# mlnoga/nightlight

Measured on AMD Instinct MI355X. Metric: stacked Mpixels/sec (sigma-clip, 128x4096x4096 fp32), higher is better.
Workload: dtype f32

## Files before the change

nightlight_amd/csrc/fast_common.hpp:

```cpp
#pragma once
#include <type_traits>
#include <utility>

#include "stack_kernels.h"

namespace nl {

constexpr float kU = 5.9604644775390625e-8f;
constexpr int kZone = 8;
constexpr int kPadMax = 8;
constexpr unsigned kGenericGrid = 2048;
inline unsigned generic_grid(unsigned hint, unsigned pixels_per_wg, unsigned max_grid)
{
    if (hint == 0) return max_grid;
    const unsigned need = (hint - 1 + pixels_per_wg - 1) / pixels_per_wg;
    const unsigned g = need + need / 2 + 64;
    return g < max_grid ? g : max_grid;
}

__device__ __forceinline__ void snapshot_fb_list(const FastArgs &q)
{
    if (q.fb_snap && threadIdx.x == 0 && __atomic_load_n(q.fb_snap, __ATOMIC_RELAXED) == 0u) {
        const unsigned len = __atomic_load_n(q.fb_count, __ATOMIC_RELAXED);
        const unsigned prev = atomicCAS(q.fb_snap, 0u, len + 1u);
        if (prev == 0xffffffffu) __builtin_trap();
        __threadfence();
    }
    __syncthreads();
}

__device__ __forceinline__ void fused_prologue_dominant(const StackArgs &p)
{
    if (p.zero_next && blockIdx.x == 0) {
        for (int i = threadIdx.x; i < kScratchWords; i += blockDim.x) p.zero_next[i] = 0ull;
        if (threadIdx.x < 4) p.final[threadIdx.x] = 0ull;
    }
}
__device__ __forceinline__ void fused_collect_slots(const StackArgs &p, unsigned block)
{
    if (p.final && block == 0 && threadIdx.x < 64) {
        unsigned long long lo = 0, hi = 0;
        for (int i = threadIdx.x; i < kClipSlots; i += 64) {
            lo += p.partial[2 * (size_t)i];
            hi += p.partial[2 * (size_t)i + 1];
        }
#pragma unroll
        for (int o = 32; o > 0; o >>= 1) {
            lo += ((unsigned long long)(unsigned)__shfl_xor((int)(lo >> 32), o, 64) << 32) | (unsigned)__shfl_xor((int)lo, o, 64);
            hi += ((unsigned long long)(unsigned)__shfl_xor((int)(hi >> 32), o, 64) << 32) | (unsigned)__shfl_xor((int)hi, o, 64);
        }
        if (threadIdx.x == 0) {
            if (lo) atomicAdd(p.final + 0, lo);
            if (hi) atomicAdd(p.final + 1, hi);
        }
    }
}
__device__ __forceinline__ unsigned long long *clip_slot(const StackArgs &p, unsigned block)
{
    return p.final ? p.final : p.partial + 2 * (size_t)(block % kClipSlots);
}

template <int B, int... I, class F>
__device__ __forceinline__ void static_for_impl(std::integer_sequence<int, I...>, F &&f)
{
    (f(std::integral_constant<int, B + I>{}), ...);
}
template <int B, int E, class F>
__device__ __forceinline__ void static_range(F &&f)
{
    if constexpr (E > B) static_for_impl<B>(std::make_integer_sequence<int, E - B>{}, static_cast<F &&>(f));
}
template <int B, int E, int CH, class F>
__device__ __forceinline__ void static_chunks(F &&f)
{
    if constexpr (E > B) {
        constexpr int M = (B + CH < E) ? B + CH : E;
        static_for_impl<B>(std::make_integer_sequence<int, M - B>{}, f);
        __builtin_amdgcn_sched_barrier(0);
        static_chunks<M, E, CH>(static_cast<F &&>(f));
    }
}
#define NL_INL __attribute__((always_inline))

struct CePair { short lo, hi; };

template <int NS>
struct OemNetwork {
    static constexpr int pow2()
    {
        int p = 1;
        while (p < NS) p <<= 1;
        return p;
    }
    static constexpr int count()
    {
        int c = 0;
        const int P2 = pow2();
        for (int p = 1; p < P2; p <<= 1)
            for (int k = p; k >= 1; k >>= 1)
                for (int j = k % p; j + k < P2; j += 2 * k)
                    for (int i = 0; i < k; i++)
                        if ((i + j) / (2 * p) == (i + j + k) / (2 * p) && (i + j + k) < NS) c++;
        return c;
    }
    static constexpr int kCount = count();
    struct Table { CePair e[kCount > 0 ? kCount : 1]; };
    static constexpr Table make()
    {
        Table t{};
        int c = 0;
        const int P2 = pow2();
        for (int p = 1; p < P2; p <<= 1)
            for (int k = p; k >= 1; k >>= 1)
                for (int j = k % p; j + k < P2; j += 2 * k)
                    for (int i = 0; i < k; i++)
                        if ((i + j) / (2 * p) == (i + j + k) / (2 * p) && (i + j + k) < NS) {
                            t.e[c].lo = (short)(i + j);
                            t.e[c].hi = (short)(i + j + k);
                            c++;
                        }
        return t;
    }
    static constexpr Table kTable = make();
};

struct FusedOp { unsigned char kind; short dst, a, b, c; };
template <int NS, int E0, int E1, int E2, int E3>
struct FusedNet;
#include "sort_tables.inc"

template <class Net, int NS, bool ASM = true, int NA = NS>
__device__ __forceinline__ void run_network(float (&v)[NA])
{
    static_assert(NS <= NA, "network larger than the column");
    float w[Net::kSlots];
    static_range<0, NS>([&](auto K) NL_INL { w[decltype(K)::value] = v[decltype(K)::value]; });
    static_chunks<0, Net::kCount, 128>([&](auto I) NL_INL {
        constexpr FusedOp op = Net::kOps[decltype(I)::value];
        float r;
        if constexpr (op.kind == 3)      r = __builtin_amdgcn_fmed3f(w[op.a], w[op.b], w[op.c]);
        else if constexpr (!ASM && op.kind == 0) r = fminf(w[op.a], w[op.b]);
        else if constexpr (!ASM && op.kind == 1) r = fmaxf(w[op.a], w[op.b]);
        else if constexpr (!ASM && op.kind == 2) r = fminf(fminf(w[op.a], w[op.b]), w[op.c]);
        else if constexpr (!ASM && op.kind == 4) r = fmaxf(fmaxf(w[op.a], w[op.b]), w[op.c]);
        else if constexpr (op.kind == 0) asm("v_min_f32 %0, %1, %2" : "=v"(r) : "v"(w[op.a]), "v"(w[op.b]));
        else if constexpr (op.kind == 1) asm("v_max_f32 %0, %1, %2" : "=v"(r) : "v"(w[op.a]), "v"(w[op.b]));
        else if constexpr (op.kind == 2) asm("v_min3_f32 %0, %1, %2, %3" : "=v"(r) : "v"(w[op.a]), "v"(w[op.b]), "v"(w[op.c]));
        else                             asm("v_max3_f32 %0, %1, %2, %3" : "=v"(r) : "v"(w[op.a]), "v"(w[op.b]), "v"(w[op.c]));
        w[op.dst] = r;
    });
    static_range<0, NS>([&](auto K) NL_INL { v[decltype(K)::value] = w[Net::kOut[decltype(K)::value]]; });
}

template <int NS, bool ASM = true, int NA = NS>
__device__ __forceinline__ void sort_network(float (&v)[NA])
{
    using Net = FusedNet<NS, 0, 0, 0, 0>;
    static_assert(Net::kComparators == OemNetwork<NS>::kCount, "sort_tables.inc does not match OemNetwork");
    run_network<Net, NS, ASM, NA>(v);
}

template <int NS, int E0, int E1, int E2, int E3>
struct ZonalNetwork {
    using Full = OemNetwork<NS>;
    static constexpr int stretch(int i) { return i < E0 ? 0 : (i < E1 ? 1 : (i < E2 ? 0 : (i < E3 ? 2 : 0))); }
    struct Table { CePair e[Full::kCount > 0 ? Full::kCount : 1]; int n; };
    static constexpr Table make()
    {
        Table t{};
        bool touched[NS] = {};
        bool keep[Full::kCount > 0 ? Full::kCount : 1] = {};
        for (int c = Full::kCount - 1; c >= 0; c--) {
            const CePair ce = Full::kTable.e[c];
            const int sl = stretch(ce.lo), sh = stretch(ce.hi);
            if (sl == sh && sl != 0 && !touched[ce.lo] && !touched[ce.hi]) continue;
            keep[c] = true;
            touched[ce.lo] = true;
            touched[ce.hi] = true;
        }
        int n = 0;
        for (int c = 0; c < Full::kCount; c++)
            if (keep[c]) t.e[n++] = Full::kTable.e[c];
        t.n = n;
        return t;
    }
    static constexpr Table kTable = make();
    static constexpr int kCount = kTable.n;
};

template <bool ASM>
struct FullSortT {
    template <int NS>
    static __device__ __forceinline__ void apply(float (&v)[NS]) { sort_network<NS, ASM>(v); }
};
using FullSort = FullSortT<true>;
template <int E0, int E1, int E2, int E3>
struct ZonalSort {
    template <int NS>
    static __device__ __forceinline__ void apply(float (&v)[NS])
    {
        using Net = FusedNet<NS, E0, E1, E2, E3>;
        static_assert(Net::kComparators == ZonalNetwork<NS, E0, E1, E2, E3>::kCount,
                      "sort_tables.inc does not match ZonalNetwork");
        run_network<Net, NS>(v);
    }
};

__device__ __forceinline__ int opaque(int x)
{
    asm volatile("" : "+v"(x));
    return x;
}

template <int B, int E, int NS>
__device__ __forceinline__ float pick(const float (&v)[NS], int idx)
{
    float r = v[B];
    static_range<B + 1, E>([&](auto K) NL_INL {
        constexpr int k = decltype(K)::value;
        if constexpr (((k - B) & 7) == 0) idx = opaque(idx);
        r = (idx == k) ? v[k] : r;
    });
    return r;
}

template <int B, int E, int NS>
__device__ __forceinline__ void pick_pair(const float (&v)[NS], int idx, float &lower, float &upper)
{
    float up = v[B], lo = v[B];
    static_range<B + 1, E>([&](auto K) NL_INL {
        constexpr int k = decltype(K)::value;
        if constexpr (((k - B) & 7) == 0) idx = opaque(idx);
        const bool hit = idx == k;
        up = hit ? v[k] : up;
        lo = hit ? v[k - 1] : lo;
    });
    upper = up;
    lower = lo;
}

__device__ __forceinline__ float max_raw(float a, float b)
{
    float r;
    asm("v_max_f32 %0, %1, %2" : "=v"(r) : "v"(a), "v"(b));
    return r;
}
__device__ __forceinline__ float min_raw(float a, float b)
{
    float r;
    asm("v_min_f32 %0, %1, %2" : "=v"(r) : "v"(a), "v"(b));
    return r;
}

__device__ __forceinline__ float nan_to_inf(float x)
{
    float y;
    asm("v_min_f32 %0, %1, %2" : "=v"(y) : "v"(x), "v"(__builtin_inff()));
    return y;
}

template <int NS, int GAP = 16, class SORT = FullSort, bool NT = false, bool PADDED = true>
__device__ __forceinline__ int gather_sorted(const float *frames, int64_t stride, int N,
                                             unsigned boff, float (&v)[NS], int lo_pads = 0)
{
    const int64_t frame_bytes = stride * (int64_t)sizeof(float);
    const int last = N - 1;
    static_chunks<0, NS / 4, 4>([&](auto C) NL_INL {
        constexpr int c0 = 4 * decltype(C)::value;
        const int f0 = min(c0, last);
        const char *gb = reinterpret_cast<const char *>(frames) + (int64_t)f0 * frame_bytes;
        const __amdgpu_buffer_rsrc_t rs =
            __builtin_amdgcn_make_buffer_rsrc(const_cast<char *>(gb), 0, -1, 0x00020000);
        static_range<0, 4>([&](auto U) NL_INL {
            constexpr int k = c0 + decltype(U)::value;
            const int soff = (min(k, last) - f0) * (int)frame_bytes;
            v[k] = __int_as_float(__builtin_amdgcn_raw_buffer_load_b32(rs, (int)boff, soff, NT ? 2 : 0));
        });
    });
    constexpr int P0 = !PADDED ? NS : (NS > GAP ? NS - GAP : 0);
    float t0 = 0.0f, t1 = 0.0f, t2 = 0.0f, t3 = 0.0f;
    static_range<P0, NS>([&](auto K) NL_INL {
        constexpr int k = decltype(K)::value;
        const int pad = (N - 1 - k) >> 31;
        const int inf = 0x7f800000 | (((k - N - lo_pads) >> 31) & (int)0x80000000);
        t0 += __int_as_float(__float_as_int(v[k]) & ~pad);
        v[k] = __int_as_float((__float_as_int(v[k]) & ~pad) | (inf & pad));
    });
    static_chunks<0, P0 / 4, 8>([&](auto K) NL_INL {
        constexpr int k = 4 * decltype(K)::value;
        t0 += v[k]; t1 += v[k + 1]; t2 += v[k + 2]; t3 += v[k + 3];
    });
    static_range<P0 / 4 * 4, P0>([&](auto K) NL_INL { t1 += v[decltype(K)::value]; });
    const float total = (t0 + t1) + (t2 + t3);
    int nan_cnt = 0;
    if (__any(!(__builtin_fabsf(total) < __builtin_inff()))) {
        static_chunks<0, NS, 8>([&](auto K) NL_INL {
            constexpr int k = decltype(K)::value;
            nan_cnt = opaque(nan_cnt - ((0x7f800000 - (__float_as_int(v[k]) & 0x7fffffff)) >> 31));
            asm volatile("v_min_f32 %0, %0, %1" : "+v"(v[k]) : "v"(__builtin_inff()));
        });
    }
    SORT::template apply<NS>(v);
    return min(N, NS) - nan_cnt;
}

struct WinsorInterval {
    float w_lo, w_hi;
    float Lm, Lp, Hm, Hp;
    float hull_lo, hull_hi;
    int guard, guard_max;
    bool ch_sure, ch_none;

    __device__ __forceinline__ void start(float s_min, float s_max, int max_rounds = 100)
    {
        guard_max = max_rounds;
        w_lo = s_min; w_hi = s_max;
        Lm = Lp = -__builtin_inff();
        Hm = Hp = __builtin_inff();
        hull_lo = __builtin_inff(); hull_hi = -__builtin_inff();
        guard = 0;
    }
    __device__ __forceinline__ void next_clamp(float median, float xmin, float xmax)
    {
        const float tA = __fmul_rn(1.5f, w_lo), tB = __fmul_rn(1.5f, w_hi);
        const float lo_m = __fsub_rn(median, tB), lo_p = __fsub_rn(median, tA);
        const float hi_m = __fadd_rn(median, tA), hi_p = __fadd_rn(median, tB);
        const float wmin_m = fmaxf(xmin, Lm), wmin_p = fmaxf(xmin, Lp);
        const float wmax_m = fminf(xmax, Hm), wmax_p = fminf(xmax, Hp);
        ch_sure = (wmin_p < lo_m) || (wmax_m > hi_p);
        ch_none = (wmin_m >= lo_p) && (wmax_p <= hi_m);
        Lm = fmaxf(Lm, lo_m); Lp = fmaxf(Lp, lo_p);
        Hm = fminf(Hm, hi_m); Hp = fminf(Hp, hi_p);
    }
    __device__ __forceinline__ void finish_round(float var_t, float err_t, float var_l, float err_l,
                                                 float eps_r, float e_m, bool shape_ok, bool &inner, bool &bail)
    {
        const float w_up = var_l + err_l;
        const float w_dn = fmaxf(var_t - err_t, 0.0f);
        const float r_hi = __builtin_amdgcn_sqrtf(w_up + w_up * eps_r + e_m * e_m) * (1.0f + 4.0f * kU) + 4.0e-19f;
        const float r_lo = __builtin_amdgcn_sqrtf(fmaxf(w_dn - w_dn * eps_r, 0.0f)) * (1.0f - 4.0f * kU);
        const float n_lo = __fmul_rn(1.134f, r_lo), n_hi = __fmul_rn(1.134f, r_hi);
        const float dmin = __fsub_rn(n_lo, w_hi), dmax = __fsub_rn(n_hi, w_lo);
        const float amin = (dmin <= 0.0f && dmax >= 0.0f) ? 0.0f : fminf(fabsf(dmin), fabsf(dmax));
        const float amx = fmaxf(fabsf(dmin), fabsf(dmax));
        const bool stop_sure = w_lo > 0.0f && amx <= w_lo * (0.0005f * (1.0f - 4.0f * kU));
        const bool go_sure = amin > w_hi * (0.0005f * (1.0f + 4.0f * kU));
        if (inner) {
            w_lo = n_lo; w_hi = n_hi;
            const bool may_stop = !ch_sure || !go_sure;
            const bool must_stop = ch_none || stop_sure;
            if (may_stop) { hull_lo = fminf(hull_lo, w_lo); hull_hi = fmaxf(hull_hi, w_hi); }
            if (!shape_ok || !(w_hi < 3.0e38f) || ++guard > guard_max) { bail = true; inner = false; }
            else if (must_stop) inner = false;
        }
    }
};

}
```

nightlight_amd/csrc/stack_fast_sigma_impl.hpp:

```cpp
#pragma once
#include "fast_ml_common.hpp"

namespace nl {


#ifndef NL_CERT_ON
#define NL_CERT_ON(ns) true
#endif
#ifndef NL_WINSOR_WL
#define NL_WINSOR_WL(ns) ((ns) >= 112 ? 20 : ((ns) >= 80 ? 16 : ((ns) / 4 + 3) / 4 * 4))
#endif

template <int NS, bool ZONAL, bool WINSOR, bool TIGHT, bool RECORD = false, bool CONT = false>
__global__ __launch_bounds__(256)
__attribute__((amdgpu_waves_per_eu((ZONAL && WINSOR && !CONT) ? (NS >= 112 ? (TIGHT ? 1 : 3) : (RECORD ? 1 : (NS >= 64 ? (TIGHT ? 4 : 1) : (NS >= 48 ? 4 : 1)))) : 1, 8)))
void stack_sigma_fast_kernel(StackArgs p, FastArgs q)
{
    static_assert(!TIGHT || ZONAL, "TIGHT is a variant of the zonal kernels");
    static_assert(!RECORD || ZONAL, "RECORD is a variant of the zonal kernels");
    static_assert(!CONT || (ZONAL && WINSOR && !RECORD), "CONT continues a winsorized zonal pass");
    constexpr bool CASCADE = ZONAL && WINSOR && !RECORD;
    if constexpr (ZONAL && !RECORD && !CONT) fused_prologue_dominant(p);
    if constexpr (!ZONAL) { if (q.in_list) { fused_collect_slots(p, blockIdx.x); snapshot_fb_list(q); } }
    constexpr int KZ = NS >= 48 ? kZone : 4, KP = TIGHT ? 0 : (NS >= 48 ? kPadMax : 4);
    static_assert(!ZONAL || NS >= 16, "zonal passes need room between the zones");
    constexpr int ZL = KZ;
    constexpr int ZH = ZONAL ? NS - KZ - KP : NS;

    int c_lo_total = 0, c_hi_total = 0;
    const bool listed = (!ZONAL || CONT) && q.in_list != nullptr;
    int64_t limit = listed ? (int64_t)min(*q.in_count, q.in_capacity) : p.npix;
    int64_t sweep = listed ? (int64_t)gridDim.x * blockDim.x : limit;
    int64_t wg_first = (int64_t)blockIdx.x * blockDim.x;
    __shared__ unsigned s_cont, s_pref[17], s_gen, s_gen_base;
    if constexpr (CASCADE) {
        if (threadIdx.x == 0) s_cont = 0u;
    }
    if constexpr (ZONAL && !RECORD) {
        if (threadIdx.x == 0) s_gen = 0u;
        __syncthreads();
    }
    if constexpr (CONT) {
        if (threadIdx.x == 0) {
            unsigned acc = 0;
            for (unsigned r = 0; r < q.in_group; r++) {
                const unsigned reg = blockIdx.x * q.in_group + r;
                s_pref[r] = acc;
                acc += reg < q.in_regions ? min(q.in_count[reg], q.in_region) : 0u;
            }
            s_pref[q.in_group] = acc;
        }
        __syncthreads();
        limit = (int64_t)s_pref[q.in_group];
        wg_first = 0;
        sweep = blockDim.x;
    } else if constexpr (CASCADE) {
        __syncthreads();
    }
    const int lane = threadIdx.x & 63;

    for (int64_t wg_item = wg_first; wg_item < limit; wg_item += sweep) {
        int N = p.n_frames;
        asm volatile("" : "+s"(N));
        const int64_t item = wg_item + threadIdx.x;
        bool on = item < limit;
        int64_t pix = item;
        unsigned cas_at = 0;
        if constexpr (CONT) {
            unsigned r = 0;
            for (unsigned k = 1; k < q.in_group; k++) r += ((unsigned)item >= s_pref[k]) ? 1u : 0u;
            cas_at = (blockIdx.x * q.in_group + r) * q.in_region + ((unsigned)item - s_pref[r]);
            pix = on ? (int64_t)q.in_list[cas_at] : 0;
        } else if (listed) pix = on ? (int64_t)q.in_list[item] : 0;
        const unsigned boff = (unsigned)(on ? pix : 0) * 4u;

        constexpr int MW0 = ZONAL ? ZH / 2 - 1 : 0, MW1 = ZONAL ? ZL + NS / 2 + 1 : NS;
        using Sorter = std::conditional_t<(ZONAL && !WINSOR && NS >= 24), ZonalSort<ZL, MW0, MW1, ZH>, FullSort>;
        float v[NS];
        int lo_pads = 0;
        if constexpr (ZONAL && !TIGHT) {
            lo_pads = min(max(KZ / 2 + 1 - (N - ZH), 0), KZ == 4 ? KZ / 2 : KZ / 2 - 1);
        }
        const int n = gather_sorted<NS, 16, Sorter, true, !TIGHT>(p.frames, p.stride, N, boff, v, lo_pads);
        bool to_exact = false;

        float res = p.ref_loc;
        int c_lo = 0, c_hi = 0;
        int a = lo_pads, b = lo_pads + n;
        bool active = on && n > 0;
        bool to_generic = false;
        if constexpr (ZONAL) {
            to_generic = active && !(b > ZH);
            active = active && !to_generic;
        }

        constexpr int W0 = ZONAL ? ZH / 2 - 1 : 0, W1 = ZONAL ? ZL + NS / 2 + 1 : NS;
        float c = pick<W0, W1>(v, a + ((b - a) >> 1));
        float d_mid = 0.0f, q_mid = 0.0f;
        if constexpr (ZONAL) {
            float d0 = 0, d1 = 0, d2 = 0, d3 = 0, q0 = 0, q1 = 0, q2 = 0, q3 = 0;
            static_chunks<0, (ZH - ZL) / 4, 4>([&](auto K) NL_INL {
                constexpr int k = ZL + 4 * decltype(K)::value;
                const float e0 = v[k] - c, e1 = v[k + 1] - c, e2 = v[k + 2] - c, e3 = v[k + 3] - c;
                d0 += e0; d1 += e1; d2 += e2; d3 += e3;
                q0 = __builtin_fmaf(e0, e0, q0); q1 = __builtin_fmaf(e1, e1, q1);
                q2 = __builtin_fmaf(e2, e2, q2); q3 = __builtin_fmaf(e3, e3, q3);
            });
            d_mid = (d0 + d1) + (d2 + d3);
            q_mid = (q0 + q1) + (q2 + q3);
        }

        constexpr int WL = ZONAL ? NL_WINSOR_WL(NS) : 0, WH = ZONAL ? NS - WL - KP : NS;
        float d_in = 0.0f, q_in = 0.0f;
        if constexpr (ZONAL && WINSOR) {
            static_assert(WL >= ZL && WH <= ZH && (WL - ZL) % 4 == 0 && (WH - WL) % 4 == 0, "winsor zones");
            float d0 = 0, d1 = 0, d2 = 0, d3 = 0, q0 = 0, q1 = 0, q2 = 0, q3 = 0;
            static_chunks<0, (WH - WL) / 4, 4>([&](auto K) NL_INL {
                constexpr int k = WL + 4 * decltype(K)::value;
                const float e0 = v[k] - c, e1 = v[k + 1] - c, e2 = v[k + 2] - c, e3 = v[k + 3] - c;
                d0 += e0; d1 += e1; d2 += e2; d3 += e3;
                q0 = __builtin_fmaf(e0, e0, q0); q1 = __builtin_fmaf(e1, e1, q1);
                q2 = __builtin_fmaf(e2, e2, q2); q3 = __builtin_fmaf(e3, e3, q3);
            });
            d_in = (d0 + d1) + (d2 + d3);
            q_in = (q0 + q1) + (q2 + q3);
        }

        if constexpr (CONT) {
            const unsigned st = on ? q.in_state[cas_at] : 0u;
            c_lo = (int)(st & 0xffffu);
            c_hi = (int)(st >> 16);
            a += c_lo;
            b -= c_hi;
        }
        int passes_left = (CASCADE && q.pass_budget > 0) ? q.pass_budget : 0x7fffffff;
        bool defer = false;

        float amax = fmaxf(fabsf(pick<0, ZONAL ? ZL : 1>(v, a)), fabsf(pick<ZONAL ? ZH : 0, NS>(v, b - 1)));

        int rnd = 0;
        if (ZONAL && lane == 0) NL_STAT(4, 1);
        auto one_pass = [&]() NL_INL {
            if constexpr (CASCADE) {
                if (passes_left <= 0) {
                    defer = defer || active;
                    active = false;
                    return;
                }
                passes_left--;
            }
            if (ZONAL) { if (lane == 0) NL_STAT(2, 1); if (active) NL_STAT(3, 1); }
            float cz = c;
            if constexpr (!ZONAL || WINSOR) asm volatile("" : "+v"(cz));
            const int cnt = b - a;
            const float fcnt = (float)cnt;
            float dz0 = 0.0f, dz1 = 0.0f, qz0 = 0.0f, qz1 = 0.0f;
            if constexpr (ZONAL) {
                static_range<0, ZL>([&](auto K) NL_INL {
                    constexpr int k = decltype(K)::value;
                    const float e = (k >= a) ? v[k] - cz : 0.0f;
                    dz0 += e;
                    qz0 = __builtin_fmaf(e, e, qz0);
                });
                static_range<ZH, NS>([&](auto K) NL_INL {
                    constexpr int k = decltype(K)::value;
                    const float e = (k < b) ? v[k] - cz : 0.0f;
                    dz1 += e;
                    qz1 = __builtin_fmaf(e, e, qz1);
                });
            } else {
                const int a1 = opaque(a);
                float dz2 = 0.0f, dz3 = 0.0f, qz2 = 0.0f, qz3 = 0.0f;
                static_chunks<0, NS / 4, 2>([&](auto K) NL_INL {
                    constexpr int k = 4 * decltype(K)::value;
                    const bool i0 = (unsigned)(k + 0 - a1) < (unsigned)cnt;
                    const bool i1 = (unsigned)(k + 1 - a1) < (unsigned)cnt;
                    const bool i2 = (unsigned)(k + 2 - a1) < (unsigned)cnt;
                    const bool i3 = (unsigned)(k + 3 - a1) < (unsigned)cnt;
                    const float e0 = i0 ? v[k + 0] - cz : 0.0f, e1 = i1 ? v[k + 1] - cz : 0.0f;
                    const float e2 = i2 ? v[k + 2] - cz : 0.0f, e3 = i3 ? v[k + 3] - cz : 0.0f;
                    dz0 += e0; dz1 += e1; dz2 += e2; dz3 += e3;
                    qz0 = __builtin_fmaf(e0, e0, qz0); qz1 = __builtin_fmaf(e1, e1, qz1);
                    qz2 = __builtin_fmaf(e2, e2, qz2); qz3 = __builtin_fmaf(e3, e3, qz3);
                });
                dz0 += dz2; dz1 += dz3; qz0 += qz2; qz1 += qz3;
            }
            const float dsum = d_mid + (dz0 + dz1);
            const float qsum = q_mid + (qz0 + qz1);
#ifdef NL_IEEE_PASS
            const float inv_cnt = 1.0f / fcnt;
            const float delta = dsum / fcnt;
#else
            const float inv_cnt = __builtin_amdgcn_rcpf(fcnt);
            const float delta = dsum * inv_cnt;
#endif
            const float m = c + delta;
#ifdef NL_IEEE_PASS
            const float aa = qsum / fcnt;
#else
            const float aa = qsum * inv_cnt;
#endif
            const float bb = delta * delta;
            const float var = fmaxf(aa - bb, 0.0f);

#ifdef NL_IEEE_PASS
            const float err_o = ((float)(NS / 2 + 24)) * kU * (aa + bb);
#else
            const float err_o = ((float)(NS / 2 + 32)) * kU * (aa + bb);
#endif
            const float eps_r = 1.02f * (fcnt + 8.0f) * kU;
            const float e_m = 1.02f * (fcnt + 2.0f) * kU * amax;
            const float v_up = var + err_o;
            const float v_dn = fmaxf(var - err_o, 0.0f);
            const float v_hi = v_up + v_up * eps_r + e_m * e_m;
            const float v_lo = fmaxf(v_dn - v_dn * eps_r, 0.0f);
#ifdef NL_IEEE_PASS
            float s_max = __fsqrt_rn(v_hi) * (1.0f + 4.0f * kU);
            float s_min = __fsqrt_rn(v_lo) * (1.0f - 4.0f * kU);
#else
            float s_max = __builtin_amdgcn_sqrtf(v_hi) * (1.0f + 6.0f * kU) + 4.0e-19f;
            float s_min = __builtin_amdgcn_sqrtf(v_lo) * (1.0f - 6.0f * kU);
#endif
            bool bail = !(v_hi < 3.0e38f);

            const int kk = a + (cnt >> 1);
            float upper, lower;
            pick_pair<W0, W1>(v, kk, lower, upper);
            const float median = (cnt & 1) ? upper : 0.5f * (lower + upper);

            float lo_min, lo_max, hi_min, hi_max;
            auto clip_counts = [&](const float smin, const float smax, int &c1, int &c2, int &d1, int &d2) NL_INL {
                const float tl0 = __fmul_rn(p.sig_lo, smin), tl1 = __fmul_rn(p.sig_lo, smax);
                const float th0 = __fmul_rn(p.sig_hi, smin), th1 = __fmul_rn(p.sig_hi, smax);
                const float la = __fsub_rn(median, tl0), lb = __fsub_rn(median, tl1);
                const float ha = __fadd_rn(median, th0), hb = __fadd_rn(median, th1);
                lo_min = fminf(la, lb); lo_max = fmaxf(la, lb);
                hi_min = fminf(ha, hb); hi_max = fmaxf(ha, hb);
                c1 = 0; c2 = 0; d1 = 0; d2 = 0;
                if constexpr (ZONAL) {
                    static_range<0, ZL>([&](auto K) NL_INL {
                        constexpr int k = decltype(K)::value;
                        c1 += (v[k] < lo_min) ? 1 : 0;
                        c2 += (v[k] < lo_max) ? 1 : 0;
                    });
                    static_range<ZH, NS>([&](auto K) NL_INL {
                        constexpr int k = decltype(K)::value;
                        d1 += (v[k] > hi_max) ? 1 : 0;
                        d2 += (v[k] > hi_min) ? 1 : 0;
                    });
                    c1 = max(c1 - a, 0); c2 = max(c2 - a, 0);
                    d1 = max(d1 - (NS - b), 0); d2 = max(d2 - (NS - b), 0);
                } else {
                    static_chunks<0, NS, 8>([&](auto K) NL_INL {
                        constexpr int k = decltype(K)::value;
                        const float x = v[k];
                        c1 += (x < lo_min) ? 1 : 0;
                        c2 += (x < lo_max) ? 1 : 0;
                        d1 += (x > hi_max) ? 1 : 0;
                        d2 += (x > hi_min) ? 1 : 0;
                    });
                    c1 = min(max(c1 - a, 0), cnt); c2 = min(max(c2 - a, 0), cnt);
                    d1 = min(max(d1 - (NS - b), 0), cnt); d2 = min(max(d2 - (NS - b), 0), cnt);
                }
            };

            if constexpr (WINSOR) {
                constexpr int PZ = ZONAL ? ZH : 0;
                const float xmin = pick<0, ZONAL ? ZL : NS>(v, a);
                const float xmax = pick<PZ, NS>(v, b - 1);
                WinsorInterval wi;
                wi.start(s_min, s_max, ((!ZONAL || CONT) && q.gen_round_cap > 0) ? q.gen_round_cap : 100);
                bool inner = active && !bail;
                int rounds_left = (CASCADE && q.round_cap > 0) ? q.round_cap : 0x7fffffff;
                constexpr bool CERT = NL_CERT_ON(NS) && (ZONAL || NS <= 32) && !RECORD;
                float wl_h0 = s_min, wl_h1 = s_min;
                int wr = 0;
                bool trial_next = false;
                while (__any(inner)) {
                    const bool is_trial = CERT && trial_next;
                    trial_next = false;
                    float Lc, Hc, ltry = 0.0f;
                    bool trial = false;
                    if (!is_trial) {
                    if constexpr (CASCADE) {
                        if (rounds_left <= 0) {
                            defer = defer || inner;
                            active = active && !inner;
                            break;
                        }
                        rounds_left--;
                    }
                    if (ZONAL) { if (lane == 0) NL_STAT(0, 1); if (inner) NL_STAT(1, 1); }
                    wl_h0 = wl_h1; wl_h1 = wi.w_lo;
                    wi.next_clamp(median, xmin, xmax);
                    Lc = wi.Lp; Hc = wi.Hm;
                    } else {
                        const float s2 = wi.w_lo, s1 = wl_h1, s0 = wl_h0;
                        const float dd1 = s1 - s2, dd0 = s0 - s1;
                        float rr = dd1 * __builtin_amdgcn_rcpf(dd0);
                        rr = fminf(fmaxf(rr, 0.0f), 0.95f);
                        const float rest = dd1 * rr * __builtin_amdgcn_rcpf(1.0f - rr);
                        ltry = fmaxf(s2 - 1.5f * rest - 1.0e-4f * s2, 0.0f);
                        trial = inner && dd1 > 0.0f && dd0 > 0.0f && ltry > 0.0f && ltry <= s2;
                        const float tq = __fmul_rn(1.5f, ltry);
                        Lc = fmaxf(wi.Lp, __fsub_rn(median, tq));
                        Hc = fminf(wi.Hm, __fadd_rn(median, tq));
                    }
                    auto clamped_variance = [&](const float Lt, const float Ht, float &wvar, float &werr, float &wmean_c,
                                                float &wrms) NL_INL {
                    float d0 = 0, d1 = 0, d2 = 0, d3 = 0, q0 = 0, q1 = 0, q2 = 0, q3 = 0;
                    if constexpr (ZONAL) {
                        static_range<0, ZL>([&](auto K) NL_INL {
                            constexpr int k = decltype(K)::value;
                            const float e = (k >= a) ? max_raw(v[k], Lt) - cz : 0.0f;
                            d0 += e; q0 = __builtin_fmaf(e, e, q0);
                        });
                        static_chunks<0, (WL - ZL) / 4, 2>([&](auto K) NL_INL {
                            constexpr int k = ZL + 4 * decltype(K)::value;
                            const float e0 = max_raw(v[k], Lt) - cz, e1 = max_raw(v[k + 1], Lt) - cz;
                            const float e2 = max_raw(v[k + 2], Lt) - cz, e3 = max_raw(v[k + 3], Lt) - cz;
                            d0 += e0; d1 += e1; d2 += e2; d3 += e3;
                            q0 = __builtin_fmaf(e0, e0, q0); q1 = __builtin_fmaf(e1, e1, q1);
                            q2 = __builtin_fmaf(e2, e2, q2); q3 = __builtin_fmaf(e3, e3, q3);
                        });
                        static_chunks<0, (ZH - WH) / 4, 2>([&](auto K) NL_INL {
                            constexpr int k = WH + 4 * decltype(K)::value;
                            const float e0 = min_raw(v[k], Ht) - cz, e1 = min_raw(v[k + 1], Ht) - cz;
                            const float e2 = min_raw(v[k + 2], Ht) - cz, e3 = min_raw(v[k + 3], Ht) - cz;
                            d0 += e0; d1 += e1; d2 += e2; d3 += e3;
                            q0 = __builtin_fmaf(e0, e0, q0); q1 = __builtin_fmaf(e1, e1, q1);
                            q2 = __builtin_fmaf(e2, e2, q2); q3 = __builtin_fmaf(e3, e3, q3);
                        });
                        static_range<ZH, NS>([&](auto K) NL_INL {
                            constexpr int k = decltype(K)::value;
                            const float e = (k < b) ? min_raw(v[k], Ht) - cz : 0.0f;
                            d1 += e; q1 = __builtin_fmaf(e, e, q1);
                        });
                        d2 += d_in; q2 += q_in;
                    } else {
                        const int a4 = opaque(a);
                        static_chunks<0, NS / 4, 2>([&](auto K) NL_INL {
                            constexpr int k = 4 * decltype(K)::value;
                            const bool i0 = (unsigned)(k + 0 - a4) < (unsigned)cnt;
                            const bool i1 = (unsigned)(k + 1 - a4) < (unsigned)cnt;
                            const bool i2 = (unsigned)(k + 2 - a4) < (unsigned)cnt;
                            const bool i3 = (unsigned)(k + 3 - a4) < (unsigned)cnt;
                            const float e0 = i0 ? __builtin_amdgcn_fmed3f(v[k + 0], Lt, Ht) - cz : 0.0f;
                            const float e1 = i1 ? __builtin_amdgcn_fmed3f(v[k + 1], Lt, Ht) - cz : 0.0f;
                            const float e2 = i2 ? __builtin_amdgcn_fmed3f(v[k + 2], Lt, Ht) - cz : 0.0f;
                            const float e3 = i3 ? __builtin_amdgcn_fmed3f(v[k + 3], Lt, Ht) - cz : 0.0f;
                            d0 += e0; d1 += e1; d2 += e2; d3 += e3;
                            q0 = __builtin_fmaf(e0, e0, q0); q1 = __builtin_fmaf(e1, e1, q1);
                            q2 = __builtin_fmaf(e2, e2, q2); q3 = __builtin_fmaf(e3, e3, q3);
                        });
                    }
                    const float wd = ((d0 + d1) + (d2 + d3)) * inv_cnt;
                    const float wa = ((q0 + q1) + (q2 + q3)) * inv_cnt;
                    const float wb = wd * wd;
                    wvar = fmaxf(wa - wb, 0.0f);
#ifdef NL_IEEE_PASS
                    werr = ((float)(NS / 2 + 34)) * kU * (wa + wb);
#else
                    werr = ((float)(NS / 2 + 40)) * kU * (wa + wb);
#endif
                    wmean_c = wd;
                    wrms = wa;
                    };
                    float var_t, err_t, wd_t, wa_t;
                    clamped_variance(Lc, Hc, var_t, err_t, wd_t, wa_t);
                    if (is_trial) {
                        const float x_dn = fmaxf(var_t - err_t, 0.0f);
                        const float x_lo = __builtin_amdgcn_sqrtf(fmaxf(x_dn - x_dn * eps_r, 0.0f)) * (1.0f - 4.0f * kU);
                        trial = trial && __fmul_rn(1.134f, x_lo) >= ltry && (!ZONAL || (v[WL] >= Lc && v[WH - 1] <= Hc));
                        const float h_lo = fminf(wi.hull_lo, ltry), h_hi = fmaxf(wi.hull_hi, wi.w_hi);
                        int e1, e2, f1, f2;
                        clip_counts(h_lo, h_hi, e1, e2, f1, f2);
                        trial = trial && e1 == e2 && f1 == f2 && h_hi < 3.0e38f;
                        if (trial) {
                            wi.hull_lo = h_lo; wi.hull_hi = h_hi;
                            inner = false;
                        }
                        continue;
                    }
                    constexpr int CS = NS >= 64 ? 4 : (NS >= 48 ? 2 : 1);
                    int t_lo = 0, t_hi = 0;
                    if constexpr (ZONAL) {
                        static_range<0, WL / CS>([&](auto J) NL_INL {
                            constexpr int k = CS * decltype(J)::value + CS - 1;
                            const bool below = v[k] < wi.Lp;
                            t_lo += ((k >= ZL || k >= a) && below) ? 1 : 0;
                        });
                        static_range<0, (NS - WH) / CS>([&](auto J) NL_INL {
                            constexpr int k = WH + CS * decltype(J)::value;
                            const bool above = v[k] > wi.Hm;
                            t_hi += ((k < ZH || k < b) && above) ? 1 : 0;
                        });
                    } else {
                        const int a5 = opaque(a);
                        static_range<0, NS / CS>([&](auto J) NL_INL {
                            constexpr int k = CS * decltype(J)::value;
                            const bool in_lo = (unsigned)(k + CS - 1 - a5) < (unsigned)cnt;
                            const bool in_hi = (unsigned)(k - a5) < (unsigned)cnt;
                            t_lo += (in_lo && v[k + CS - 1] < wi.Lp) ? 1 : 0;
                            t_hi += (in_hi && v[k] > wi.Hm) ? 1 : 0;
                        });
                    }
                    float var_l, err_l;
                    {
                        const float n_lo = (float)min(CS * t_lo + CS - 1 - (a % CS), cnt);
                        const float n_hi = (float)min(CS * t_hi + ((b - 1) % CS), cnt);
                        const float dL = (wi.Lp - wi.Lm) * (1.0f + 2.0f * kU), dH = (wi.Hp - wi.Hm) * (1.0f + 2.0f * kU);
                        const float ybar = cz + wd_t;
                        const float slop = 4.0e-6f * __builtin_amdgcn_sqrtf(wa_t) + 4.0f * kU * fabsf(ybar) + 1.0e-30f;
                        const float gL = fmaxf(ybar - wi.Lp, 0.0f) + slop, gH = fmaxf(wi.Hm - ybar, 0.0f) + slop;
                        const float corr = (n_lo * (dL * (2.0f * gL + dL)) + n_hi * (dH * (2.0f * gH + dH))) * inv_cnt;
                        var_l = var_t + ((corr == corr) ? corr * 1.001f : 0.0f);
                        err_l = err_t;
                    }
                    const bool shape_ok = !ZONAL || (v[WL] >= wi.Lp && v[WH - 1] <= wi.Hm);
                    wi.finish_round(var_t, err_t, var_l, err_l, eps_r, e_m, shape_ok, inner, bail);
                    wr++;
                    if constexpr (CERT) trial_next = q.cert_first > 0 && wr >= q.cert_first && ((wr - q.cert_first) % q.cert_every) == 0;
                }
                s_min = wi.hull_lo;
                s_max = wi.hull_hi;
            }

            int c1, c2, d1, d2;
            clip_counts(s_min, s_max, c1, c2, d1, d2);
            if constexpr (ZONAL) {
                if (active && ((a + c2 >= ZL) || (b - d2 <= ZH))) {
                    to_generic = true;
                    active = false;
                }
            }
            if (active) {
                bail |= (c1 != c2) || (d1 != d2) || (lo_max > hi_min && (c1 + d1) > 0);
                if (bail) {
                    to_exact = true;
                    active = false;
                    if constexpr (WINSOR && !RECORD) { if (p.nrounds) p.nrounds[pix] = (unsigned char)(ZONAL ? min(rnd, kBoundRounds) : 0); }
                } else {
                    if constexpr (WINSOR && ZONAL && !RECORD) {
                        if (p.bounds) {
                            if (rnd < kBoundRounds) p.bounds[(size_t)rnd * (size_t)p.npix + (size_t)pix] = make_float2(lo_max, hi_min);
                            rnd++;
                        }
                    }
                    if constexpr (RECORD) {
                        if (rnd < kBoundRounds) p.bounds[(size_t)rnd * (size_t)p.npix + (size_t)pix] = make_float2(lo_max, hi_min);
                        rnd++;
                    }
                    c_lo += c1;
                    c_hi += d1;
                    a += c1;
                    b -= d1;
                    amax = fminf(amax, fmaxf(fabsf(lo_min), fabsf(hi_max)));
                    if ((c1 + d1) == 0 || (b - a) <= 1) {
                        res = m;
                        active = false;
                    }
                }
            }
        };
        auto flush = [&]() NL_INL {
        if (on && !active && !to_generic && !to_exact && !defer) {
            NL_STORE_RESULT(&p.out[pix], res);
            c_lo_total += c_lo;
            c_hi_total += c_hi;
        }
        if constexpr (CASCADE) {
            const unsigned long long dm = __ballot(on && defer);
            if (dm) {
                unsigned base = 0;
                if (lane == 0) base = atomicAdd(&s_cont, (unsigned)__popcll(dm));
                base = __shfl(base, 0, 64);
                const unsigned slot = base + (unsigned)__popcll(dm & ((1ull << lane) - 1ull));
                if (on && defer && slot < q.cont_region) {
                    const size_t at = (size_t)blockIdx.x * q.cont_region + slot;
                    q.cont_list[at] = (unsigned)pix;
                    q.cont_state[at] = (unsigned)c_lo | ((unsigned)c_hi << 16);
                }
            }
        }
        if constexpr (ZONAL && !RECORD) {
            const unsigned long long gm = __ballot(on && to_generic);
            unsigned woff = 0;
            if (lane == 0 && gm) woff = atomicAdd(&s_gen, (unsigned)__popcll(gm));
            __syncthreads();
            if (threadIdx.x == 0) s_gen_base = s_gen ? atomicAdd(q.gen_count, s_gen) : 0u;
            __syncthreads();
            if (gm) {
                const unsigned base = s_gen_base + (unsigned)__shfl((int)woff, 0, 64);
                const unsigned slot = base + (unsigned)__popcll(gm & ((1ull << lane) - 1ull));
                if (on && to_generic && slot < q.gen_capacity) q.gen_list[slot] = (unsigned)pix;
            }
            __syncthreads();
            if (threadIdx.x == 0) s_gen = 0u;
        }
        const unsigned long long em = RECORD ? 0ull : __ballot(on && to_exact);
        if (em) {
            unsigned base = 0;
            if (lane == 0) base = atomicAdd(q.fb_count, (unsigned)__popcll(em));
            base = __shfl(base, 0, 64);
            const unsigned slot = base + (unsigned)__popcll(em & ((1ull << lane) - 1ull));
            if (on && to_exact && slot < q.fb_capacity) q.fb_list[slot] = (unsigned)pix;
        }
            on = on && active;
            to_generic = false;
            to_exact = false;
            defer = false;
        };
        while (__any(active)) one_pass();
        if constexpr (RECORD) {
            const bool decided = on && !to_generic && !to_exact && n > 0 && rnd <= kBoundRounds;
            if (on) p.nrounds[pix] = (unsigned char)(decided ? rnd : 0);
        } else {
            flush();
        }
    }
    if constexpr (RECORD) return;
    if constexpr (CASCADE) {
        if (q.cont_count) {
            __syncthreads();
            if (threadIdx.x == 0) q.cont_count[blockIdx.x] = min(s_cont, q.cont_region);
        }
    }

    __shared__ int s_lo[4], s_hi[4];
#pragma unroll
    for (int o = 32; o > 0; o >>= 1) {
        c_lo_total += __shfl_xor(c_lo_total, o, 64);
        c_hi_total += __shfl_xor(c_hi_total, o, 64);
    }
    if ((threadIdx.x & 63) == 0) { s_lo[threadIdx.x >> 6] = c_lo_total; s_hi[threadIdx.x >> 6] = c_hi_total; }
    __syncthreads();
    if (threadIdx.x == 0) {
        int t_lo = 0, t_hi = 0;
        for (unsigned w = 0; w < (blockDim.x >> 6); w++) { t_lo += s_lo[w]; t_hi += s_hi[w]; }
        unsigned long long *slot = p.partial + 2 * (size_t)(blockIdx.x % kClipSlots);
        if constexpr (!ZONAL) slot = clip_slot(p, blockIdx.x);
        if (t_lo) atomicAdd(slot + 0, (unsigned long long)t_lo);
        if (t_hi) atomicAdd(slot + 1, (unsigned long long)t_hi);
    }
}


}
```

Before: 10120.

## Use prefix-sum tables and binary mux trees in zonal non-winsor sigma-clip passes

For zonal kernels without winsorization, the code now precomputes suffix and prefix sums of deviations and squared deviations over the low and high zones once per pixel. Each pass then reads them through a binary select tree indexed by the bits of the cut positions, instead of re-summing the zones with predicated loops. Clip counts come from a branchless binary-search rank over the sorted zone values, and the median pair is fetched with a mux tree rather than a linear select chain. The cost is extra registers for the tables, which may lower occupancy, and the per-pass control flow is rewritten, which could change edge-case behaviour.

```diff
diff --git a/nightlight_amd/csrc/fast_common.hpp b/nightlight_amd/csrc/fast_common.hpp
--- a/nightlight_amd/csrc/fast_common.hpp
+++ b/nightlight_amd/csrc/fast_common.hpp
@@ -237,6 +237,49 @@
     });
     upper = up;
     lower = lo;
+}
+
+constexpr int ilog2_ceil(int n) { return n <= 1 ? 0 : 1 + ilog2_ceil((n + 1) / 2); }
+constexpr int ilog2_exact(int n) { return (1 << ilog2_ceil(n)) == n ? ilog2_ceil(n) : -1; }
+
+template <int NB, int LO, int BASE = 0, int M, class F>
+__device__ __forceinline__ float mux_tree(const bool (&bit)[M], F &&leaf)
+{
+    if constexpr (NB == 0) {
+        return leaf(std::integral_constant<int, BASE>{});
+    } else {
+        const float hi = mux_tree<NB - 1, LO + 1, BASE + (1 << LO)>(bit, leaf);
+        const float lo = mux_tree<NB - 1, LO + 1, BASE>(bit, leaf);
+        return bit[LO] ? hi : lo;
+    }
+}
+
+template <int M>
+__device__ __forceinline__ void index_bits(int idx, bool (&bit)[M])
+{
+    static_range<0, M>([&](auto I) NL_INL {
+        constexpr int i = decltype(I)::value;
+        bit[i] = i == M - 1 ? idx >= (1 << i) : (idx & (1 << i)) != 0;
+    });
+}
+
+template <int M, class Z, class P>
+__device__ __forceinline__ int zone_rank(Z &&z, P &&pred, bool &full, float &last)
+{
+    bool bit[M];
+    float lst = 0.0f;
+    int r = 0;
+    static_range<0, M>([&](auto L) NL_INL {
+        constexpr int l = decltype(L)::value;
+        const float x = mux_tree<l, M - l>(bit, [&](auto B) NL_INL { return z(std::integral_constant<int, decltype(B)::value + (1 << (M - 1 - l)) - 1>{}); });
+        const bool hit = pred(x);
+        bit[M - 1 - l] = hit;
+        lst = hit ? x : lst;
+        r += hit ? (1 << (M - 1 - l)) : 0;
+    });
+    full = pred(z(std::integral_constant<int, (1 << M) - 1>{}));
+    last = lst;
+    return r;
 }
 
 __device__ __forceinline__ float max_raw(float a, float b)
diff --git a/nightlight_amd/csrc/stack_fast_sigma_impl.hpp b/nightlight_amd/csrc/stack_fast_sigma_impl.hpp
--- a/nightlight_amd/csrc/stack_fast_sigma_impl.hpp
+++ b/nightlight_amd/csrc/stack_fast_sigma_impl.hpp
@@ -109,6 +109,30 @@
             d_mid = (d0 + d1) + (d2 + d3);
             q_mid = (q0 + q1) + (q2 + q3);
         }
+        constexpr bool ZT = ZONAL && !WINSOR;
+        constexpr int ZHW = NS - ZH;
+        constexpr int ML = ZT ? ilog2_exact(ZL) : 0, MH = ZT ? ilog2_exact(ZHW) : 0;
+        float tdl[ZT ? ZL : 1], tql[ZT ? ZL : 1], tdh[ZT ? ZHW : 1], tqh[ZT ? ZHW : 1];
+        if constexpr (ZT) {
+            float sd = 0.0f, sq = 0.0f;
+            static_range<0, ZL>([&](auto K) NL_INL {
+                constexpr int k = ZL - 1 - decltype(K)::value;
+                const float e = v[k] - c;
+                sd += e;
+                sq = __builtin_fmaf(e, e, sq);
+                tdl[k] = sd;
+                tql[k] = sq;
+            });
+            sd = 0.0f; sq = 0.0f;
+            static_range<ZH, NS>([&](auto K) NL_INL {
+                constexpr int k = decltype(K)::value;
+                const float e = v[k] - c;
+                sd += e;
+                sq = __builtin_fmaf(e, e, sq);
+                tdh[NS - 1 - k] = sd;
+                tqh[NS - 1 - k] = sq;
+            });
+        }
 
         constexpr int WL = ZONAL ? NL_WINSOR_WL(NS) : 0, WH = ZONAL ? NS - WL - KP : NS;
         float d_in = 0.0f, q_in = 0.0f;
@@ -155,7 +179,15 @@
             const int cnt = b - a;
             const float fcnt = (float)cnt;
             float dz0 = 0.0f, dz1 = 0.0f, qz0 = 0.0f, qz1 = 0.0f;
-            if constexpr (ZONAL) {
+            if constexpr (ZT) {
+                bool ba[ML], bb[MH];
+                index_bits(a, ba);
+                index_bits(NS - b, bb);
+                dz0 = mux_tree<ML, 0>(ba, [&](auto J) NL_INL { return tdl[decltype(J)::value]; });
+                qz0 = mux_tree<ML, 0>(ba, [&](auto J) NL_INL { return tql[decltype(J)::value]; });
+                dz1 = mux_tree<MH, 0>(bb, [&](auto J) NL_INL { return tdh[decltype(J)::value]; });
+                qz1 = mux_tree<MH, 0>(bb, [&](auto J) NL_INL { return tqh[decltype(J)::value]; });
+            } else if constexpr (ZONAL) {
                 static_range<0, ZL>([&](auto K) NL_INL {
                     constexpr int k = decltype(K)::value;
                     const float e = (k >= a) ? v[k] - cz : 0.0f;
@@ -208,8 +240,8 @@
 #else
             const float err_o = ((float)(NS / 2 + 32)) * kU * (aa + bb);
 #endif
-            const float eps_r = 1.02f * (fcnt + 8.0f) * kU;
-            const float e_m = 1.02f * (fcnt + 2.0f) * kU * amax;
+            const float eps_r = (fcnt + 8.0f) * (1.02f * kU);
+            const float e_m = (fcnt + 2.0f) * (1.02f * kU) * amax;
             const float v_up = var + err_o;
             const float v_dn = fmaxf(var - err_o, 0.0f);
             const float v_hi = v_up + v_up * eps_r + e_m * e_m;
@@ -225,17 +257,29 @@
 
             const int kk = a + (cnt >> 1);
             float upper, lower;
-            pick_pair<W0, W1>(v, kk, lower, upper);
+            if constexpr (ZT) {
+                constexpr int K0 = (ZH + 1) / 2, K1 = (ZL - 1 + NS) / 2, MK = ilog2_ceil(K1 - K0 + 1);
+                static_assert(K0 - 1 >= W0 && K1 < W1, "the median window holds exact ranks");
+                bool bk[MK];
+                index_bits(kk - K0, bk);
+                upper = mux_tree<MK, 0>(bk, [&](auto J) NL_INL { constexpr int j = decltype(J)::value; return v[K0 + (j < K1 - K0 ? j : K1 - K0)]; });
+                lower = mux_tree<MK, 0>(bk, [&](auto J) NL_INL { constexpr int j = decltype(J)::value; return v[K0 - 1 + (j < K1 - K0 ? j : K1 - K0)]; });
+            } else {
+                pick_pair<W0, W1>(v, kk, lower, upper);
+            }
             const float median = (cnt & 1) ? upper : 0.5f * (lower + upper);
 
             float lo_min, lo_max, hi_min, hi_max;
-            auto clip_counts = [&](const float smin, const float smax, int &c1, int &c2, int &d1, int &d2) NL_INL {
+            auto thresholds = [&](const float smin, const float smax) NL_INL {
                 const float tl0 = __fmul_rn(p.sig_lo, smin), tl1 = __fmul_rn(p.sig_lo, smax);
                 const float th0 = __fmul_rn(p.sig_hi, smin), th1 = __fmul_rn(p.sig_hi, smax);
                 const float la = __fsub_rn(median, tl0), lb = __fsub_rn(median, tl1);
                 const float ha = __fadd_rn(median, th0), hb = __fadd_rn(median, th1);
                 lo_min = fminf(la, lb); lo_max = fmaxf(la, lb);
                 hi_min = fminf(ha, hb); hi_max = fmaxf(ha, hb);
+            };
+            auto clip_counts = [&](const float smin, const float smax, int &c1, int &c2, int &d1, int &d2) NL_INL {
+                thresholds(smin, smax);
                 c1 = 0; c2 = 0; d1 = 0; d2 = 0;
                 if constexpr (ZONAL) {
                     static_range<0, ZL>([&](auto K) NL_INL {
@@ -426,16 +470,60 @@
                 s_max = wi.hull_hi;
             }
 
-            int c1, c2, d1, d2;
-            clip_counts(s_min, s_max, c1, c2, d1, d2);
+            int c1, d1;
+            bool overflow, undecided;
+            if constexpr (ZT) {
+                {
+                    const float la = __fsub_rn(median, __fmul_rn(p.sig_lo, s_min)), lb = __fsub_rn(median, __fmul_rn(p.sig_lo, s_max));
+                    const float ha = __fadd_rn(median, __fmul_rn(p.sig_hi, s_min)), hb = __fadd_rn(median, __fmul_rn(p.sig_hi, s_max));
+                    lo_min = min_raw(la, lb); lo_max = max_raw(la, lb);
+                    hi_min = min_raw(ha, hb); hi_max = max_raw(ha, hb);
+                }
+                const int u = NS - b;
+                bool full_lo, full_hi;
+                float last_lo, last_hi;
+                const int r_lo = zone_rank<ML>([&](auto J) NL_INL { return v[decltype(J)::value]; },
+                                               [&](float x) NL_INL { return x < lo_max; }, full_lo, last_lo);
+                const int r_hi = zone_rank<MH>([&](auto J) NL_INL { return v[NS - 1 - decltype(J)::value]; },
+                                               [&](float x) NL_INL { return x > hi_min; }, full_hi, last_hi);
+                overflow = full_lo || full_hi;
+                c1 = max(r_lo - a, 0);
+                d1 = max(r_hi - u, 0);
+                undecided = (c1 > 0 && !(last_lo < lo_min)) || (d1 > 0 && !(last_hi > hi_max));
+            } else {
+                int c2, d2;
+                clip_counts(s_min, s_max, c1, c2, d1, d2);
+                overflow = ZONAL && ((a + c2 >= ZL) || (b - d2 <= ZH));
+                undecided = (c1 != c2) || (d1 != d2);
+            }
+            if constexpr (ZT) {
+                const bool gen = active && overflow;
+                const bool exact = active && !overflow && (bail || undecided || (lo_max > hi_min && (c1 + d1) > 0));
+                const bool step = active && !gen && !exact;
+                if constexpr (RECORD) {
+                    if (step && rnd < kBoundRounds) p.bounds[(size_t)rnd * (size_t)p.npix + (size_t)pix] = make_float2(lo_max, hi_min);
+                    rnd += step ? 1 : 0;
+                }
+                c1 = step ? c1 : 0;
+                d1 = step ? d1 : 0;
+                a += c1;
+                b -= d1;
+                amax = min_raw(amax, max_raw(fabsf(lo_min), fabsf(hi_max)));
+                const bool done = step && ((c1 + d1) == 0 || (b - a) <= 1);
+                res = done ? m : res;
+                to_generic = to_generic || gen;
+                to_exact = to_exact || exact;
+                active = step && !done;
+                return;
+            }
             if constexpr (ZONAL) {
-                if (active && ((a + c2 >= ZL) || (b - d2 <= ZH))) {
+                if (active && overflow) {
                     to_generic = true;
                     active = false;
                 }
             }
             if (active) {
-                bail |= (c1 != c2) || (d1 != d2) || (lo_max > hi_min && (c1 + d1) > 0);
+                bail |= undecided || (lo_max > hi_min && (c1 + d1) > 0);
                 if (bail) {
                     to_exact = true;
                     active = false;
@@ -516,6 +604,10 @@
             const bool decided = on && !to_generic && !to_exact && n > 0 && rnd <= kBoundRounds;
             if (on) p.nrounds[pix] = (unsigned char)(decided ? rnd : 0);
         } else {
+            if constexpr (ZT) {
+                c_lo = a - lo_pads;
+                c_hi = lo_pads + n - b;
+            }
             flush();
         }
     }
```

After: 10600 (median of 6 runs). +4.8%, better.
